# PimLb/POMDP_PBVI_Exploration

Measured on AMD Instinct MI355X. Metric: alpha-vector backups/sec, higher is better.
Workload: dtype f32

## Files before the change

### include/pbvi_hip.h

```cpp
#ifndef PBVI_HIP_H
#define PBVI_HIP_H

#include <stddef.h>
#include <stdint.h>

#ifdef __cplusplus
extern "C" {
#endif

typedef struct pbvi_engine pbvi_engine_t;

enum pbvi_status {
    PBVI_OK = 0,
    PBVI_EINVAL = -1,
    PBVI_ENOMEM = -2,
    PBVI_ERUNTIME = -3,
    PBVI_EUNSUPPORTED = -4
};

enum pbvi_dtype { PBVI_F32 = 0, PBVI_F64 = 1 };

enum pbvi_mode {
    PBVI_SPARSE = 0,
    PBVI_DENSE = 1
// ... 160 lines not shown
                             int32_t* out_steps , uint8_t* out_lost );

int pbvi_mdp_value_iteration(int device, int32_t S, int32_t A, int32_t R, const int32_t* reach_states,
                             const double* reach_prob, const double* exp_reward, const double* v0, double gamma,
                             double max_change_limit, int32_t horizon, double* out_rows, double* out_changes,
                             int32_t* out_iterations);

int64_t pbvi_belief_walk(pbvi_engine_t* e, const double* b0, int64_t n, const int32_t* actions, const int32_t* observations,
                         const uint8_t* restart, double* out_beliefs);
int pbvi_belief_walk_keys(pbvi_engine_t* e, int64_t n, uint64_t* out_keys);
int pbvi_engine_set_rto_f64(pbvi_engine_t* e, const double* rto);

int pbvi_set_formulation(pbvi_engine_t* e, int formulation);

int pbvi_set_f64_screen(pbvi_engine_t* e, int mode);

int pbvi_set_fused_projection(pbvi_engine_t* e, int enable);

int pbvi_set_score_split(pbvi_engine_t* e, int mode);

int pbvi_set_gamma_tiling(pbvi_engine_t* e, int mode, int64_t chunk_rows);
int pbvi_gamma_tiling_plan(int32_t S, int32_t A, int32_t O, int64_t V, int64_t B, int dtype, int64_t budget_bytes,
                           int64_t* chunk_rows, int64_t* n_chunks, int64_t* bytes_needed);

int pbvi_set_tie_window(pbvi_engine_t* e, double rel);

int pbvi_debug_poison(int enable);
int64_t pbvi_debug_alloc_limit(int64_t mb);
int pbvi_engine_after_oom(pbvi_engine_t* e);
int64_t pbvi_debug_live_bytes(void);

int pbvi_debug_gemm_dense(int enable);
int pbvi_debug_split_schedule(int schedule);
int64_t pbvi_debug_slabs(pbvi_engine_t* e, void* out, int64_t cap_bytes);
int pbvi_debug_slabs_fill(pbvi_engine_t* e, int byte);
int pbvi_debug_score_probe(pbvi_engine_t* e, int enable);
int pbvi_debug_score_probe_fetch(pbvi_engine_t* e, int64_t* dims, double* scalars, double* score, double* mag, double* E,
                                 int32_t* best_v, double* best_score, int32_t* queue, uint8_t* dead, int32_t* perm);
int pbvi_debug_refine_counts(pbvi_engine_t* e, int64_t out[8]);
int pbvi_debug_value_max_route(pbvi_engine_t* e, int64_t out[8]);

int64_t pbvi_device_bytes(const pbvi_engine_t* e);

#ifdef __cplusplus
}
#endif
#endif
```

### pomdp_pbvi_exploration_amd/csrc/engine.hip

```cpp
#include <algorithm>
#include <atomic>
#include <cmath>
#include <cstddef>
#include <cstdio>
#include <cstdlib>
#include <cstring>
#include <condition_variable>
#include <mutex>
#include <new>
#include <string>
#include <thread>
#include <unistd.h>
#include <vector>

#include "backup_kernels.h"
#include "split_bf16.h"
#include "upper_kernels.h"

namespace pbvi {

static thread_local std::string g_err;
static int g_poison = -1;
static bool poison_enabled() {
    if (g_poison < 0) g_poison = getenv("PBVI_POISON") != nullptr ? 1 : 0;
// ... 4528 lines not shown
}
int64_t pbvi_backup_unique_count(const pbvi_engine_t* e) { return (e && e->impl) ? e->impl->unique_count() : -1; }
int pbvi_backup_fetch_unique(pbvi_engine_t* e, void* out_rows, int32_t* out_index) {
    NEED(e);
    return e->impl->fetch_unique(out_rows, out_index);
}
int pbvi_backup_run_fetch(pbvi_engine_t* e, double gamma, int flags, pbvi_stats_t* stats, void* out_rows, int64_t cap_rows,
                          int32_t* out_slot, int32_t* out_index, int32_t* out_action, int32_t* out_best_alpha, uint8_t* out_keep,
                          int64_t* n_unique, int64_t* n_slots) {
    NEED(e);
    return e->impl->run_fetch(gamma, flags, stats, out_rows, cap_rows, out_slot, out_index, out_action, out_best_alpha, out_keep,
                              n_unique, n_slots);
}
int pbvi_backup_fetch_compact(pbvi_engine_t* e, void* out_rows, int32_t* out_index, int32_t* out_action,
                              int32_t* out_best_alpha, uint8_t* out_keep) {
    NEED(e);
    return e->impl->fetch_compact(out_rows, out_index, out_action, out_best_alpha, out_keep);
}
void* pbvi_host_alloc(size_t bytes) {
    void* p = nullptr;
    if (bytes == 0) return nullptr;
    if (hipHostMalloc(&p, bytes, hipHostMallocDefault) != hipSuccess) {
        (void)hipGetLastError();
        pbvi::set_error("pbvi_host_alloc: hipHostMalloc of " + std::to_string(bytes) + " bytes failed");
        return nullptr;
    }
    return p;
}
void pbvi_host_free(void* p) {
    if (p && hipHostFree(p) != hipSuccess) (void)hipGetLastError();
}
int pbvi_debug_gemm_dense(int enable) { return pbvi::set_gemm_force_dense(enable); }
int pbvi_debug_split_schedule(int schedule) { return pbvi::set_gemm_split_schedule(schedule); }
int64_t pbvi_debug_slabs(pbvi_engine_t* e, void* out, int64_t cap_bytes) {
    NEED(e);
    return e->impl->debug_slabs(out, cap_bytes);
}
int pbvi_debug_slabs_fill(pbvi_engine_t* e, int byte) {
    NEED(e);
    return e->impl->debug_slabs_fill(byte);
}
int pbvi_debug_score_probe(pbvi_engine_t* e, int enable) {
    NEED(e);
    return e->impl->debug_score_probe(enable);
}
int pbvi_debug_refine_counts(pbvi_engine_t* e, int64_t out[8]) {
    NEED(e);
    return e->impl->debug_refine_counts(out);
}
int pbvi_debug_value_max_route(pbvi_engine_t* e, int64_t out[8]) {
    NEED(e);
    return e->impl->debug_value_max_route(out);
}
int pbvi_debug_score_probe_fetch(pbvi_engine_t* e, int64_t* dims, double* scalars, double* score, double* mag, double* err,
                                 int32_t* best_v, double* best_score, int32_t* queue, uint8_t* dead, int32_t* perm) {
    NEED(e);
    return e->impl->debug_score_probe_fetch(dims, scalars, score, mag, err, best_v, best_score, queue, dead, perm);
}
int pbvi_backup(pbvi_engine_t* e, const void* beliefs, int64_t B, double gamma, int flags, void* out_alpha,
                int32_t* out_action, int32_t* out_best_alpha, uint8_t* out_keep, pbvi_stats_t* stats) {
    NEED(e);
    int rc = e->impl->beliefs_set(beliefs, B);
    if (rc) return rc;
    rc = e->impl->backup_run(gamma, flags, stats);
    if (rc) return rc;
    return e->impl->backup_fetch(out_alpha, out_action, out_best_alpha, out_keep);
// ... 262 lines not shown
```

### pomdp_pbvi_exploration_amd/csrc/gemm.hip

```cpp
#include "pbvi_common.h"
#include "split_bf16.h"

#include <cstdlib>
#include <map>
#include <mutex>

namespace pbvi {

typedef float f32x4 __attribute__((ext_vector_type(4)));
typedef float f32x16 __attribute__((ext_vector_type(16)));

constexpr int TILE_FLOATS = 256 * GEMM_BK;
constexpr int KL_IRR_BIT = 30;
constexpr int KL_MASK = (1 << KL_IRR_BIT) - 1;
constexpr int GEMM_LDS_BYTES = 4 * TILE_FLOATS * 4;

__device__ __forceinline__ void glds16(const float* g, float* l) {
    __builtin_amdgcn_global_load_lds((const __attribute__((address_space(1))) void*)g,
                                     (__attribute__((address_space(3))) void*)l, 16, 0, 0);
}

struct TileThread {
    int lane, wid, i, h, wr, wc;
    int srow[4], scol[4];
    int a_row[4], b_row[2];
    __device__ __forceinline__ void init() {
        const int tid = threadIdx.x;
        lane = tid & 63;
        wid = __builtin_amdgcn_readfirstlane(tid >> 6);
        i = lane & 31;
        h = lane >> 5;
        wr = wid >> 2;
        wc = wid & 3;
#pragma unroll
        for (int it = 0; it < 4; ++it) {
            const int c = it * 512 + tid;
// ... 613 lines not shown
}
__device__ __forceinline__ void split_read_b(const TileThread& t, const float* lds, int buf, int kk, bool lo, i32x4 (&b)[2]) {
    const uint32_t addr = lds_addr(lds + buf * 2 * TILE_FLOATS + TILE_FLOATS + t.wc * 64 * GEMM_BK) + split_lane_part(t, kk, lo);
    lds_read16(b[0], addr, 0);
    lds_read16(b[1], addr, 32 * GEMM_BK * 4);
}
#define PBVI_SPLIT_WAIT(N) "s_waitcnt lgkmcnt(" #N ")"
#define PBVI_SPLIT_A(a) "+v"(a[0]), "+v"(a[1]), "+v"(a[2]), "+v"(a[3])
#define PBVI_SPLIT_B(b) "+v"(b[0]), "+v"(b[1])
#define split_wait_ab(N, a, b)                                                            \
    do {                                                                                  \
        asm volatile(PBVI_SPLIT_WAIT(N) : PBVI_SPLIT_A(a), PBVI_SPLIT_B(b)::"memory");    \
        __builtin_amdgcn_sched_barrier(0);                                                \
    } while (0)
#define split_wait_a(N, a)                                              \
    do {                                                                \
        asm volatile(PBVI_SPLIT_WAIT(N) : PBVI_SPLIT_A(a)::"memory");   \
        __builtin_amdgcn_sched_barrier(0);                              \
    } while (0)
#define split_wait_b(N, b)                                              \
    do {                                                                \
        asm volatile(PBVI_SPLIT_WAIT(N) : PBVI_SPLIT_B(b)::"memory");   \
        __builtin_amdgcn_sched_barrier(0);                              \
    } while (0)
__device__ __forceinline__ void split_mfma8(const i32x4 (&a)[4], const i32x4 (&b)[2], f32x16 (&acc)[4][2]) {
#pragma unroll
    for (int mi = 0; mi < 4; ++mi)
#pragma unroll
        for (int ni = 0; ni < 2; ++ni)
            acc[mi][ni] = __builtin_amdgcn_mfma_f32_32x32x16_bf16(__builtin_bit_cast(bf16x8, a[mi]), __builtin_bit_cast(bf16x8, b[ni]),
                                                                  acc[mi][ni], 0, 0, 0);
}

template <int SCHED>
__device__ __forceinline__ void tile_run_split(const TileThread& t, float* lds, const float* Aplane, int lda, const float* Bblk,
                                               int ldb, bool gen, const int32_t* __restrict__ rsrow,
                                               const float* __restrict__ rtorow, const float* __restrict__ arow0,
                                               int64_t a_step, float gamma, const int* __restrict__ kl, int i0, int i1,
                                               f32x16 (&acc)[4][2]) {
    const int tid = threadIdx.x;
    const int kg = tid & 3, r0 = tid >> 2;
    f32x4 xb[2][2];
    i32x4 idx[2];
    f32x4 w[2];
    const uint32_t a_off = (uint32_t)(t.srow[0] * lda + t.scol[0]) * 4u;
    auto stage_a = [&](int buf, int entry) {
        const char* base = (const char*)(Aplane + (int64_t)(entry & KL_MASK) * GEMM_BK);
        float* la = lds + buf * 2 * TILE_FLOATS;
#pragma unroll
        for (int it = 0; it < 4; ++it)
            glds16((const float*)(base + (int64_t)it * 64 * lda * 4 + a_off), la + (it * 512 + t.wid * 64) * 4);
    };
    auto load_rows = [&](int entry) {
        const int k = (entry & KL_MASK) * GEMM_BK + kg * 8;
#pragma unroll
        for (int it = 0; it < 2; ++it) {
            const float* p = Bblk + (int64_t)(it * 128 + r0) * ldb + k;
            ld16(xb[it][0], p);
            ld16(xb[it][1], p + 4);
        }
    };
    auto indices = [&](int entry) {
        const int s = (entry & KL_MASK) * GEMM_BK + kg * 8;
        ld16i(idx[0], rsrow + s);
        ld16i(idx[1], rsrow + s + 4);
    };
    auto weights = [&](int entry) {
        const int s = (entry & KL_MASK) * GEMM_BK + kg * 8;
        ld16(w[0], rtorow + s);
        ld16(w[1], rtorow + s + 4);
    };
    auto alphas = [&](int entry) {
        if (entry >> KL_IRR_BIT) {
// ... 25 lines not shown
        float* lb = lds + buf * 2 * TILE_FLOATS + TILE_FLOATS;
        if (gen)
            split_store(lb, it * 128 + r0, kg, fused_value(gamma, w[0], xb[it][0]), fused_value(gamma, w[1], xb[it][1]));
        else
            split_store(lb, it * 128 + r0, kg, xb[it][0], xb[it][1]);
    };
    auto wait_and_store_b0 = [&](int buf) {
        if (gen)
            asm volatile("s_waitcnt vmcnt(6)" : "+v"(xb[0][0]), "+v"(xb[0][1]), "+v"(xb[1][0]), "+v"(xb[1][1]), "+v"(w[0]),
                         "+v"(w[1])::"memory");
        else
            asm volatile("s_waitcnt vmcnt(4)" : "+v"(xb[0][0]), "+v"(xb[0][1]), "+v"(xb[1][0]), "+v"(xb[1][1])::"memory");
        store_b(buf, 0);
    };
    {
        const int e0 = kl[i0];
        if (gen) {
            indices(e0);
            weights(e0);
            asm volatile("s_waitcnt vmcnt(0)" : "+v"(idx[0]), "+v"(idx[1])::"memory");
            alphas(e0);
            indices(i0 + 1 < i1 ? kl[i0 + 1] : 0);
        } else {
            load_rows(e0);
        }
        stage_a(0, e0);
        asm volatile("s_waitcnt vmcnt(0)" : "+v"(xb[0][0]), "+v"(xb[0][1]), "+v"(xb[1][0]), "+v"(xb[1][1]), "+v"(w[0]), "+v"(w[1]),
                     "+v"(idx[0]), "+v"(idx[1])::"memory");
        store_b(0, 0);
        store_b(0, 1);
    }
    int k_next = (i0 + 1 < i1) ? kl[i0 + 1] : 0;
    int k_after = (i0 + 2 < i1) ? kl[i0 + 2] : 0;
    __syncthreads();
    int buf = 0;
    for (int it = i0; it < i1; ++it) {
        int k_after2 = 0;
        const bool more = it + 1 < i1;
        if (more) {
            if (gen) {
                alphas(k_next);
                weights(k_next);
                indices(k_after);
            } else {
                load_rows(k_next);
            }
            stage_a(buf ^ 1, k_next);
            if (it + 3 < i1) k_after2 = kl[it + 3];
        }
        if constexpr (SCHED == SPLIT_SCHED_PIPELINED) {
            SplitSlots f;
            split_read_a(t, lds, buf, 0, false, f.a[0]);
            split_read_b(t, lds, buf, 0, false, f.b[0]);
            split_read_b(t, lds, buf, 0, true, f.b[1]);
            split_wait_ab(2, f.a[0], f.b[0]);
            split_mfma8(f.a[0], f.b[0], acc);
            __builtin_amdgcn_sched_barrier(0);
            split_read_a(t, lds, buf, 0, true, f.a[1]);
            split_wait_b(4, f.b[1]);
            split_mfma8(f.a[0], f.b[1], acc);
            __builtin_amdgcn_sched_barrier(0);
            split_read_a(t, lds, buf, 1, false, f.a[0]);
            split_read_b(t, lds, buf, 1, false, f.b[1]);
            split_wait_a(6, f.a[1]);
            split_mfma8(f.a[1], f.b[0], acc);
            __builtin_amdgcn_sched_barrier(0);
            split_read_b(t, lds, buf, 1, true, f.b[0]);
            split_wait_ab(2, f.a[0], f.b[1]);
            split_mfma8(f.a[0], f.b[1], acc);
            __builtin_amdgcn_sched_barrier(0);
            split_read_a(t, lds, buf, 1, true, f.a[1]);
            split_wait_b(4, f.b[0]);
            if (more) wait_and_store_b0(buf ^ 1);
            split_mfma8(f.a[0], f.b[0], acc);
            __builtin_amdgcn_sched_barrier(0);
            split_wait_a(0, f.a[1]);
            if (more) store_b(buf ^ 1, 1);
            split_mfma8(f.a[1], f.b[1], acc);
        } else {
            SplitFrag f;
            split_group(t, lds, buf, 0, 0, f, acc);
            split_group(t, lds, buf, 0, 1, f, acc);
            split_group(t, lds, buf, 0, 2, f, acc);
            split_group(t, lds, buf, 1, 0, f, acc);
            if (more) wait_and_store_b0(buf ^ 1);
            split_group(t, lds, buf, 1, 1, f, acc);
            if (more) store_b(buf ^ 1, 1);
            split_group(t, lds, buf, 1, 2, f, acc);
        }
        asm volatile("s_waitcnt vmcnt(0)" : "+v"(idx[0]), "+v"(idx[1])::"memory");
        __syncthreads();
        buf ^= 1;
        k_next = k_after;
        k_after = k_after2;
    }
}

template <int SCHED>
__device__ __forceinline__ void gemm_split_streamk_body(const float* __restrict__ A, int lda, const float* __restrict__ B, int ldb,
                                                        FusedB fb, SlabOut out, StreamKView v) {
    extern __shared__ __attribute__((aligned(16))) float lds[];
    streamk_walk(v, out, [&](const TileThread& t, int p, int tm, int tn, int lo, int hi, auto& acc) {
        const float* Ablk = A + (int64_t)tm * 256 * lda;
        if (fb.mat == nullptr || fb.mat[tn]) {
            const int bt = (fb.mat != nullptr && fb.ctile != nullptr) ? fb.ctile[tn] : tn;
            tile_run_split<SCHED>(t, lds, Ablk, lda, B + (int64_t)bt * 256 * ldb, ldb, false, nullptr, nullptr, nullptr, 0,
                                  0.f, v.klist + (int64_t)p * v.k_tiles, lo, hi, acc);
        } else {
            const int r0 = tn * 256;
            const int g = r0 / fb.V, v0 = r0 - g * fb.V;
            tile_run_split<SCHED>(t, lds, Ablk, lda, nullptr, 0, true, fb.rs + (int64_t)(g / fb.O) * fb.S_pad,
                                  fb.rto + (int64_t)g * fb.S_pad, fb.alpha + (int64_t)(v0 + (threadIdx.x >> 2)) * fb.lda,
                                  (int64_t)128 * fb.lda, fb.gamma, v.klist + (int64_t)p * v.k_tiles, lo, hi, acc);
        }
    });
}

__global__ __launch_bounds__(512) void k_gemm_split_streamk(
    const float* __restrict__ A, int lda, const float* __restrict__ B, int ldb, FusedB fb, float* __restrict__ C, int ldc,
    int64_t slab_stride, int tiles_m, int pairs, int k_tiles, const int* __restrict__ klist, const int* __restrict__ kcount,
    const int* __restrict__ prefix, const int* __restrict__ start_pair, const int* __restrict__ first_block,
    const int* __restrict__ plan, int ovh) {
    gemm_split_streamk_body<SPLIT_SCHED_PARENT>(A, lda, B, ldb, fb, SlabOut{C, ldc, slab_stride},
        StreamKView{klist, kcount, prefix, start_pair, first_block, plan, tiles_m, pairs, k_tiles, ovh});
}
__global__ __launch_bounds__(512) void k_gemm_split_streamk_pipelined(
    const float* __restrict__ A, int lda, const float* __restrict__ B, int ldb, FusedB fb, float* __restrict__ C, int ldc,
    int64_t slab_stride, int tiles_m, int pairs, int k_tiles, const int* __restrict__ klist, const int* __restrict__ kcount,
    const int* __restrict__ prefix, const int* __restrict__ start_pair, const int* __restrict__ first_block,
    const int* __restrict__ plan, int ovh) {
    gemm_split_streamk_body<SPLIT_SCHED_PIPELINED>(A, lda, B, ldb, fb, SlabOut{C, ldc, slab_stride},
        StreamKView{klist, kcount, prefix, start_pair, first_block, plan, tiles_m, pairs, k_tiles, ovh});
}

__global__ void k_split_probe(float* out) {
    const int lane = threadIdx.x, r = lane & 31, h = lane >> 5;
    float a[8] = {0.f, 0.f, 0.f, 0.f, 0.f, 0.f, 0.f, 0.f}, b[8] = {0.f, 0.f, 0.f, 0.f, 0.f, 0.f, 0.f, 0.f};
    const float x = 0x1.02p-120f + 0x1p-132f;
    if (h == 0) {
        a[0] = x;
        a[1] = 0x1p-100f;
        if (r == 0) b[0] = 1.f;
        if (r == 1) b[1] = 0x1p-30f;
    }
    i32x4 ah, al, bh, bl;
    uint32_t hh, ll;
#pragma unroll
    for (int p = 0; p < 4; ++p) {
        split_pair(a[2 * p], a[2 * p + 1], hh, ll); ah[p] = (int)hh; al[p] = (int)ll;
        split_pair(b[2 * p], b[2 * p + 1], hh, ll); bh[p] = (int)hh; bl[p] = (int)ll;
    }
    f32x16 acc;
#pragma unroll
    for (int e = 0; e < 16; ++e) acc[e] = 0.f;
    acc = __builtin_amdgcn_mfma_f32_32x32x16_bf16(__builtin_bit_cast(bf16x8, ah), __builtin_bit_cast(bf16x8, bh), acc, 0, 0, 0);
    acc = __builtin_amdgcn_mfma_f32_32x32x16_bf16(__builtin_bit_cast(bf16x8, ah), __builtin_bit_cast(bf16x8, bl), acc, 0, 0, 0);
    acc = __builtin_amdgcn_mfma_f32_32x32x16_bf16(__builtin_bit_cast(bf16x8, al), __builtin_bit_cast(bf16x8, bh), acc, 0, 0, 0);
    if (lane < 2) out[lane] = acc[0];
    if (lane == 0) out[2] = x;
}

int gemm_split_supported(int device) {
    static std::mutex mu;
    static std::map<int, int> known;
// ... 70 lines not shown
            if (nzB == nullptr) {
                f = 1;
            } else if (G == 0) {
                f = nzB[((int64_t)batch * tiles_n + tn) * k_tiles + kt];
            } else {
                for (int g = g0; g <= g1; ++g) f |= nzB[(int64_t)g * k_tiles + kt];
            }
        }
        const unsigned long long mask = __ballot(f);
        if (lane == 0) wcount[wid] = __popcll(mask);
        __syncthreads();
        int off = total;
        for (int w = 0; w < wid; ++w) off += wcount[w];
        if (f) {
            int entry = kt;
            if (irr != nullptr && g0 == g1 && g1 < G && irr[(int64_t)(g0 / groups_per_action) * k_tiles + kt]) entry |= 1 << KL_IRR_BIT;
            klist[(int64_t)pair * k_tiles + off + __popcll(mask & ((1ull << lane) - 1ull))] = entry;
        }
        __syncthreads();
        if (tid == 0) total += wcount[0] + wcount[1] + wcount[2] + wcount[3];
        __syncthreads();
    }
    if (tid == 0) {
        kcount[pair] = total;
        nchunks[pair] = (total + chunk_len - 1) / chunk_len;
    }
}

struct GemmEnv {
    int dense;
    int chunk;
    int no_streamk;
    int ovh;
};
static int env_int(const char* name, int dflt) { return getenv(name) ? atoi(getenv(name)) : dflt; }
static const GemmEnv& gemm_env() {
    static const GemmEnv env{env_int("PBVI_GEMM_DENSE", 0) != 0, env_int("PBVI_GEMM_CHUNK", 0), env_int("PBVI_GEMM_NO_STREAMK", 0),
                             env_int("PBVI_STREAMK_OVH", 1)};
    return env;
}

static int g_force_dense = -1;
int gemm_force_dense() { return g_force_dense < 0 ? gemm_env().dense : g_force_dense; }
int set_gemm_force_dense(int enable) {
    const int prev = gemm_force_dense();
    g_force_dense = enable ? 1 : 0;
    return prev;
}

static int g_split_schedule = SPLIT_SCHED_PARENT;
int set_gemm_split_schedule(int schedule) {
    const int prev = g_split_schedule;
    if (schedule == SPLIT_SCHED_PARENT || schedule == SPLIT_SCHED_PIPELINED) g_split_schedule = schedule;
    return prev;
}

int choose_chunk_len(int tiles_mn, int k_tiles) {
    if (const int v = gemm_env().chunk; v > 0) return v < k_tiles ? v : k_tiles;
    const int64_t total = (int64_t)tiles_mn * k_tiles;
    int64_t len = total / (256 * 8);
    if (len < 8) len = 8;
    if (len > 96) len = 96;
    if (len > k_tiles) len = k_tiles;
    return (int)len;
}

static int device_cu_count() {
    static int cus = 0;
    if (cus == 0) {
        int dev = 0;
        hipDeviceProp_t prop;
        if (hipGetDevice(&dev) == hipSuccess && hipGetDeviceProperties(&prop, dev) == hipSuccess)
            cus = prop.multiProcessorCount;
        if (cus <= 0) cus = 256;
    }
    return cus;
}

hipError_t launch_tile_nonzero_f32(const float* X, int ld, int rows_pad, int k_tiles, uint8_t* nz, hipStream_t stream) {
    dim3 grid((k_tiles + 7) / 8, rows_pad / 256);
    hipLaunchKernelGGL(k_tile_nonzero, grid, dim3(256), 0, stream, X, ld, k_tiles, nz);
    return hipGetLastError();
}

using StreamKKernel = void (*)(const float*, int, const float*, int, FusedB, float*, int, int64_t, int, int, int, const int*,
                               const int*, const int*, const int*, const int*, const int*, int);
struct StreamKKernelRow {
    int split, schedule, fused, R;
    StreamKKernel kernel;
    int lds_bytes;
};
constexpr int ANY = -1;
static const StreamKKernelRow STREAMK_KERNELS[] = {
    {1, SPLIT_SCHED_PARENT, ANY, ANY, k_gemm_split_streamk, GEMM_LDS_BYTES},
    {1, SPLIT_SCHED_PIPELINED, ANY, ANY, k_gemm_split_streamk_pipelined, GEMM_LDS_BYTES},
    {0, ANY, 0, ANY, k_gemm_nt_f32_streamk, GEMM_LDS_BYTES},
    {0, ANY, 1, 1, k_gemm_nt_f32_streamk_fused, GEMM_LDS_BYTES},
    {0, ANY, 1, 2, k_gemm_nt_f32_streamk_fused_r<2>, GEMM_LDS_BYTES_R},
    {0, ANY, 1, 3, k_gemm_nt_f32_streamk_fused_r<3>, GEMM_LDS_BYTES_R},
    {0, ANY, 1, 4, k_gemm_nt_f32_streamk_fused_r<4>, GEMM_LDS_BYTES_R},
    {0, ANY, 1, 5, k_gemm_nt_f32_streamk_fused_r<5>, GEMM_LDS_BYTES_R},
    {0, ANY, 1, 6, k_gemm_nt_f32_streamk_fused_r<6>, GEMM_LDS_BYTES_R},
    {0, ANY, 1, 7, k_gemm_nt_f32_streamk_fused_r<7>, GEMM_LDS_BYTES_R},
};
static const StreamKKernelRow* streamk_kernel(int split, int schedule, int fused, int R) {
    auto fits = [](int want, int have) { return want == ANY || want == have; };
    for (const StreamKKernelRow& row : STREAMK_KERNELS)
        if (fits(row.split, split) && fits(row.schedule, schedule) && fits(row.fused, fused) && fits(row.R, R)) return &row;
    return nullptr;
}

static hipError_t set_lds_attr() {
    static bool done = false;
    if (done) return hipSuccess;
    hipError_t e = hipFuncSetAttribute((const void*)k_gemm_nt_f32_mfma, hipFuncAttributeMaxDynamicSharedMemorySize,
                                       GEMM_LDS_BYTES);
    for (const StreamKKernelRow& row : STREAMK_KERNELS)
        if (e == hipSuccess) e = hipFuncSetAttribute((const void*)row.kernel, hipFuncAttributeMaxDynamicSharedMemorySize, row.lds_bytes);
    done = e == hipSuccess;
    return e;
}

static hipError_t build_klists(const GemmArgs& a, int batch, const FusedB* fused, hipStream_t ls) {
    if (batch < 1 || batch > 65535) return hipErrorInvalidValue;
    const GemmPlan& pl = a.plan;
    hipLaunchKernelGGL(k_build_klists, dim3(pl.tiles_m * pl.tiles_n, batch), dim3(256), 0, ls, a.nzA, a.nzB, a.G, a.v_group,
                       a.n_rows, pl.tiles_m, pl.k_tiles, pl.chunk_len, gemm_force_dense(), a.klist, a.kcount, a.nchunks,
                       fused != nullptr ? fused->irr : nullptr, fused != nullptr ? fused->O : 1);
    return hipGetLastError();
}

static hipError_t launch_mfma(const GemmArgs& a, int batch, int64_t batch_stride_b, int64_t batch_stride_c) {
    const GemmPlan& pl = a.plan;
    const int64_t groups = ((int64_t)pl.tiles_n * pl.max_chunks + 7) / 8 * 8;
    const int64_t total = groups * pl.tiles_m;
    if (total <= 0 || total > 0x7fffffff) return hipErrorInvalidValue;
    hipLaunchKernelGGL(k_gemm_nt_f32_mfma, dim3((unsigned)total, batch), dim3(512), GEMM_LDS_BYTES, a.stream, a.A, a.lda, a.B,
                       a.ldb, a.C, pl.ldc, pl.slab_stride, pl.tiles_m, pl.tiles_n, pl.k_tiles, pl.chunk_len, pl.max_chunks,
                       a.klist, a.kcount, batch_stride_b, batch_stride_c);
    return hipGetLastError();
}

hipError_t launch_score_gemm_f32(const ScoreGemmArgs& a) {
    hipError_t e = set_lds_attr();
    if (e != hipSuccess) return e;
    const GemmPlan& pl = a.plan;
    const int fused_R = a.fused != nullptr ? a.fused->R : 1;
    if (pl.streamk ? a.streamk_ws == nullptr : (a.fused != nullptr || a.split)) return hipErrorInvalidValue;
    if (a.split && fused_R != 1) return hipErrorInvalidValue;
    hipStream_t ls = (a.list_stream != nullptr && a.list_event != nullptr) ? a.list_stream : a.stream;
    if ((e = build_klists(a, 1, a.fused, ls)) != hipSuccess) return e;
    const int pairs = pl.tiles_m * pl.tiles_n, ovh = gemm_env().ovh;
    const StreamKWorkspace ws = streamk_workspace(pl, a.streamk_ws);
    if (pl.streamk) {
        hipLaunchKernelGGL(k_streamk_plan, dim3(1), dim3(256), 0, ls, a.kcount, pairs, pl.nblocks, pl.k_tiles, pl.max_chunks - 1,
                           ovh, ws.prefix, ws.start_pair, ws.first_block, a.nchunks, ws.plan);
        if ((e = hipGetLastError()) != hipSuccess) return e;
    }
    if (ls != a.stream) {
        if ((e = hipEventRecord(a.list_event, ls)) != hipSuccess) return e;
        if ((e = hipStreamWaitEvent(a.stream, a.list_event, 0)) != hipSuccess) return e;
    }
    if (!pl.streamk) return launch_mfma(a, 1, 0, 0);
    const StreamKKernelRow* row = streamk_kernel(a.split ? 1 : 0, g_split_schedule, a.fused != nullptr, fused_R);
    if (row == nullptr) return hipErrorInvalidValue;
    const FusedB fb = a.fused != nullptr ? *a.fused : FusedB{};
    hipLaunchKernelGGL(row->kernel, dim3(pl.nblocks), dim3(512), row->lds_bytes, a.stream, a.A, a.lda, a.B, a.ldb, fb, a.C, pl.ldc,
                       pl.slab_stride, pl.tiles_m, pairs, pl.k_tiles, a.klist, a.kcount, ws.prefix, ws.start_pair, ws.first_block,
                       ws.plan, ovh);
    return hipGetLastError();
}

hipError_t launch_batched_gemm_f32(const BatchedGemmArgs& a) {
    hipError_t e = set_lds_attr();
    if (e != hipSuccess) return e;
    if (a.plan.streamk) return hipErrorInvalidValue;
    if ((e = build_klists(a, a.batch, nullptr, a.stream)) != hipSuccess) return e;
    if (a.ev_before != nullptr && (e = hipEventRecord(a.ev_before, a.stream)) != hipSuccess) return e;
    if ((e = launch_mfma(a, a.batch, a.batch_stride_b, a.batch_stride_c)) != hipSuccess) return e;
    if (a.ev_after != nullptr && (e = hipEventRecord(a.ev_after, a.stream)) != hipSuccess) return e;
    return hipSuccess;
}

GemmPlan make_gemm_plan(int M_pad, int N_pad, int K_pad, bool single_chunk) {
    GemmPlan pl;
    pl.tiles_m = M_pad / GEMM_BM;
    pl.tiles_n = N_pad / GEMM_BN;
    pl.k_tiles = K_pad / GEMM_BK;
    pl.ldc = N_pad;
    pl.slab_stride = (int64_t)M_pad * N_pad;
    pl.streamk = !single_chunk && !gemm_env().no_streamk;
    pl.nblocks = device_cu_count();
    if (single_chunk) {
        pl.chunk_len = pl.k_tiles;
        pl.max_chunks = 1;
    } else if (pl.streamk) {
        const int max_split = 8;
// ... 47 lines not shown
```

### pomdp_pbvi_exploration_amd/csrc/pbvi_common.h

```cpp
#pragma once
#include <hip/hip_runtime.h>
#include <stdint.h>
#include <string>

#include "../../include/pbvi_hip.h"

namespace pbvi {

void set_error(const std::string& msg);

constexpr int GEMM_BM = 256;
constexpr int GEMM_BN = 256;
constexpr int GEMM_BK = 32;

inline int64_t round_up(int64_t x, int64_t m) { return (x + m - 1) / m * m; }

struct GemmPlan {
    int tiles_m, tiles_n, k_tiles, chunk_len, max_chunks, ldc;
    int64_t slab_stride;
    bool streamk;
    int nblocks;
    int64_t c_floats;
};
int set_gemm_force_dense(int enable);
int set_gemm_split_schedule(int schedule);
int gemm_force_dense();
struct StreamKWorkspace {
    int *prefix, *start_pair, *first_block, *plan;
};
inline StreamKWorkspace streamk_workspace(const GemmPlan& pl, int* ws, size_t* ints = nullptr) {
    const size_t pairs = (size_t)pl.tiles_m * pl.tiles_n;
    size_t off = 0;
    auto take = [&](size_t n) {
        int* p = ws != nullptr ? ws + off : nullptr;
        off += n;
        return p;
    };
    const StreamKWorkspace w{take(pairs + 1), take((size_t)pl.nblocks), take(pairs), take(2)};
    if (ints != nullptr) *ints = off;
    return w;
}
inline size_t streamk_workspace_ints(const GemmPlan& pl) {
    size_t n = 0;
    streamk_workspace(pl, nullptr, &n);
    return n;
}
struct FusedB {
    const float* alpha;
    int lda;
    const int32_t* rs;
    const float* rto;
    int S_pad, O, V;
    int R;
    float gamma;
    const int32_t* ctile;
    const uint8_t* mat;
    const int32_t* irr;
// ... 54 lines not shown
```

### pomdp_pbvi_exploration_amd/engine.py

```python
from __future__ import annotations

import ctypes as C
import os
from dataclasses import dataclass

import numpy as np

PKG_DIR = os.path.dirname(os.path.abspath(__file__))
LIB_PATH = os.path.join(PKG_DIR, 'libpbvi_hip.so')

PBVI_F32, PBVI_F64 = 0, 1
PBVI_SPARSE, PBVI_DENSE = 0, 1
PBVI_BELIEF_DOMINANCE = 1

EXPORTS = [
    'pbvi_version', 'pbvi_device_count', 'pbvi_last_error', 'pbvi_engine_create', 'pbvi_engine_destroy',
    'pbvi_alpha_set', 'pbvi_alpha_append', 'pbvi_alpha_count', 'pbvi_beliefs_set', 'pbvi_backup_run',
    'pbvi_backup_fetch', 'pbvi_backup_unique_count', 'pbvi_backup_fetch_unique', 'pbvi_backup_device_results',
    'pbvi_backup', 'pbvi_prune_dominated', 'pbvi_value_max',
    'pbvi_set_tie_window', 'pbvi_device_bytes',
    'pbvi_alpha_store_append', 'pbvi_alpha_select', 'pbvi_alpha_store_reset',
    'pbvi_belief_store_append', 'pbvi_beliefs_select', 'pbvi_belief_store_reset', 'pbvi_debug_poison',
    'pbvi_belief_update', 'pbvi_beliefs_advance', 'pbvi_beliefs_fetch', 'pbvi_beliefs_count',
    'pbvi_mdp_value_iteration', 'pbvi_set_formulation', 'pbvi_belief_walk', 'pbvi_engine_set_rto_f64', 'pbvi_backup_fetch_unique_keys', 'pbvi_assemble_rows',
    'pbvi_backup_fetch_exchange', 'pbvi_backup_store_unique',
    'pbvi_value_max_store', 'pbvi_belief_store_count', 'pbvi_alpha_store_count', 'pbvi_set_value_max_exact', 'pbvi_alpha_layout',
    'pbvi_belief_walk_keys', 'pbvi_backup_fetch_value_max',
    'pbvi_backup_fetch_compact', 'pbvi_host_alloc', 'pbvi_host_free', 'pbvi_debug_gemm_dense',
    'pbvi_backup_fetch_exchange_padded', 'pbvi_assemble_rows_store', 'pbvi_exchange_merge', 'pbvi_backup_run_fetch', 'pbvi_debug_alloc_limit', 'pbvi_debug_live_bytes', 'pbvi_engine_after_oom', 'pbvi_set_f64_screen', 'pbvi_set_fused_projection', 'pbvi_backup_fetch_row_hashes', 'pbvi_set_score_split',
    'pbvi_set_gamma_tiling', 'pbvi_gamma_tiling_plan', 'pbvi_q_values', 'pbvi_prune_dominated_masked',
    'pbvi_rollout', 'pbvi_infotaxis', 'pbvi_rollout_infotaxis', 'pbvi_debug_split_schedule', 'pbvi_debug_slabs',
    'pbvi_debug_slabs_fill', 'pbvi_env_set_frames', 'pbvi_env_set_table', 'pbvi_env_clear', 'pbvi_rollout_env',
    'pbvi_debug_score_probe', 'pbvi_debug_score_probe_fetch', 'pbvi_debug_refine_counts', 'pbvi_debug_value_max_route',
    'pbvi_upper_reset', 'pbvi_upper_append', 'pbvi_upper_count', 'pbvi_upper_bound', 'pbvi_upper_q',
    'pbvi_state_weights_set', 'pbvi_state_weights_clear', 'pbvi_space_aware', 'pbvi_rollout_space_aware',
]


class EngineUnavailable(RuntimeError):
    """The HIP library is missing or no GPU is visible."""


class PbviStats(C.Structure):
    _fields_ = [('ms_total', C.c_double), ('ms_project', C.c_double), ('ms_score', C.c_double),
                ('ms_argmax', C.c_double), ('ms_refine', C.c_double), ('ms_action', C.c_double),
                ('ms_assemble', C.c_double), ('ms_dominance', C.c_double), ('n_pairs', C.c_int64),
                ('n_dead', C.c_int64), ('n_refined', C.c_int64), ('n_refined_actions', C.c_int64),
                ('n_unique', C.c_int64),
                ('score_flops', C.c_int64), ('score_flops_executed', C.c_int64), ('score_tiles_dense', C.c_int64),
                ('score_tiles_run', C.c_int64), ('project_flops', C.c_int64), ('project_flops_executed', C.c_int64),
                ('split_k', C.c_int32), ('formulation', C.c_int32), ('n_refine_candidates', C.c_int64),
                ('ms_project_gemm', C.c_double), ('screened', C.c_int32), ('fused_projection', C.c_int32),
                ('score_split', C.c_int32), ('gamma_chunks', C.c_int32)]

    def as_dict(self) -> dict:
        return {name: getattr(self, name) for name, _ in self._fields_}


_lib = None


def load_library(path: str = LIB_PATH):
    global _lib
    if _lib is not None:
        return _lib
    path = os.environ.get('PBVI_LIB_PATH', path)
    if not os.path.exists(path):
        raise EngineUnavailable(f'{path} not found: build it with `python -m pomdp_pbvi_exploration_amd.build`')
    try:
        lib = C.CDLL(path)
    except OSError as e:
        raise EngineUnavailable(f'cannot load {path}: {e}') from e
    vp, i32p, u8p, f64p = C.c_void_p, C.POINTER(C.c_int32), C.POINTER(C.c_uint8), C.POINTER(C.c_double)
    sp = C.POINTER(PbviStats)
    protos = {
        'pbvi_version': (C.c_int, []),
        'pbvi_device_count': (C.c_int, []),
        'pbvi_last_error': (C.c_char_p, []),
        'pbvi_engine_create': (C.c_int, [C.POINTER(vp), C.c_int, C.c_int32, C.c_int32, C.c_int32, C.c_int32,
                                         i32p, vp, vp, C.c_int, C.c_int]),
        'pbvi_engine_destroy': (None, [vp]),
        'pbvi_alpha_set': (C.c_int, [vp, vp, C.c_int64]),
        'pbvi_alpha_append': (C.c_int, [vp, vp, C.c_int64]),
        'pbvi_alpha_count': (C.c_int64, [vp]),
        'pbvi_beliefs_set': (C.c_int, [vp, vp, C.c_int64]),
        'pbvi_backup_run': (C.c_int, [vp, C.c_double, C.c_int, sp]),
        'pbvi_backup_fetch': (C.c_int, [vp, vp, i32p, i32p, u8p]),
        'pbvi_backup_unique_count': (C.c_int64, [vp]),
        'pbvi_backup_fetch_unique': (C.c_int, [vp, vp, i32p]),
        'pbvi_backup_fetch_compact': (C.c_int, [vp, vp, i32p, i32p, i32p, u8p]),
        'pbvi_host_alloc': (vp, [C.c_size_t]),
        'pbvi_host_free': (None, [vp]),
        'pbvi_debug_gemm_dense': (C.c_int, [C.c_int]),
        'pbvi_debug_split_schedule': (C.c_int, [C.c_int]),
        'pbvi_debug_slabs': (C.c_int64, [vp, vp, C.c_int64]),
        'pbvi_debug_slabs_fill': (C.c_int, [vp, C.c_int]),
        'pbvi_debug_score_probe': (C.c_int, [vp, C.c_int]),
        'pbvi_debug_score_probe_fetch': (C.c_int, [vp] + [vp] * 10),
        'pbvi_debug_refine_counts': (C.c_int, [vp, vp]),
        'pbvi_debug_value_max_route': (C.c_int, [vp, vp]),
        'pbvi_backup_store_unique': (C.c_int64, [vp, i32p, C.c_int64]),
        'pbvi_backup_device_results': (C.c_int, [vp, C.POINTER(vp), C.POINTER(vp), C.POINTER(vp)]),
        'pbvi_backup': (C.c_int, [vp, vp, C.c_int64, C.c_double, C.c_int, vp, i32p, i32p, u8p, sp]),
        'pbvi_prune_dominated': (C.c_int, [vp, u8p]),
        'pbvi_prune_dominated_masked': (C.c_int, [vp, u8p, u8p]),
        'pbvi_value_max': (C.c_int, [vp, f64p, i32p]),
        'pbvi_value_max_store': (C.c_int, [vp, C.c_int64, f64p, i32p]),
        'pbvi_q_values': (C.c_int, [vp, C.c_double, f64p, i32p, i32p]),
        'pbvi_belief_store_count': (C.c_int64, [vp]),
        'pbvi_backup_fetch_value_max': (C.c_int, [vp, f64p]),
        'pbvi_belief_walk_keys': (C.c_int, [vp, C.c_int64, C.POINTER(C.c_uint64)]),
        'pbvi_set_value_max_exact': (C.c_int, [vp, C.c_int]),
        'pbvi_alpha_layout': (C.c_int, [vp, C.POINTER(C.c_int64), C.POINTER(C.c_int64)]),
        'pbvi_alpha_store_count': (C.c_int64, [vp]),
        'pbvi_alpha_store_append': (C.c_int64, [vp, vp, C.c_int64]),
        'pbvi_alpha_select': (C.c_int, [vp, i32p, C.c_int64]),
        'pbvi_alpha_store_reset': (C.c_int, [vp]),
        'pbvi_belief_store_append': (C.c_int64, [vp, vp, C.c_int64]),
        'pbvi_beliefs_select': (C.c_int, [vp, i32p, C.c_int64]),
        'pbvi_belief_store_reset': (C.c_int, [vp]),
        'pbvi_debug_poison': (C.c_int, [C.c_int]),
        'pbvi_belief_update': (C.c_int, [vp, i32p, i32p, vp]),
        'pbvi_beliefs_advance': (C.c_int, [vp, i32p, i32p, u8p, C.POINTER(C.c_int64)]),
        'pbvi_rollout': (C.c_int, [vp, i32p, C.c_int, C.c_double, i32p, u8p, C.c_uint64, C.c_uint64, C.c_int64,
                                   i32p, i32p, i32p, i32p]),
        'pbvi_infotaxis': (C.c_int, [vp, f64p, i32p, f64p, f64p]),
        'pbvi_rollout_infotaxis': (C.c_int, [vp, i32p, u8p, C.c_uint64, C.c_uint64, C.c_int64, i32p, i32p, i32p, i32p]),
# ... 55 lines not shown
def debug_alloc_limit(mb: int) -> int:
    return int(load_library().pbvi_debug_alloc_limit(int(mb)))


def debug_live_bytes() -> int:
    return int(load_library().pbvi_debug_live_bytes())


def gamma_tiling_plan(S: int, A: int, O: int, V: int, B: int, dtype: str = 'f32', budget_bytes: int = 0,
                      chunk_rows: int = 0) -> tuple:
    if dtype not in ('f32', 'f64'):
        raise ValueError("dtype must be 'f32' or 'f64'")
    for name, v in (('S', S), ('A', A), ('O', O)):
        if not -2**31 <= int(v) < 2**31:
            raise ValueError(f'{name} out of range')
    rows, n, need = C.c_int64(int(chunk_rows)), C.c_int64(0), C.c_int64(0)
    _check(load_library().pbvi_gamma_tiling_plan(int(S), int(A), int(O), int(V), int(B), 0 if dtype == 'f32' else 1,
                                                 int(budget_bytes), C.byref(rows), C.byref(n), C.byref(need)))
    return int(rows.value), int(n.value), int(need.value)


def debug_gemm_dense(enable: bool) -> bool:
    return bool(load_library().pbvi_debug_gemm_dense(1 if enable else 0))


SPLIT_SCHEDULES = {'parent': 0, 'pipelined': 1}


def debug_split_schedule(schedule: str) -> str:
    prev = int(load_library().pbvi_debug_split_schedule(SPLIT_SCHEDULES[schedule]))
    return {v: k for k, v in SPLIT_SCHEDULES.items()}[prev]


def device_count() -> int:
    return int(load_library().pbvi_device_count())


class _PinnedArray(np.ndarray):

    def __array_finalize__(self, obj):
        self._owner = getattr(obj, '_owner', None)


class PinnedBuffer:

    def __init__(self, nbytes: int):
        self._lib = load_library()
        self.nbytes = int(nbytes)
        self._p = self._lib.pbvi_host_alloc(self.nbytes)
        if not self._p:
            raise MemoryError((self._lib.pbvi_last_error() or b'').decode(errors='replace'))
        self._raw = (C.c_uint8 * self.nbytes).from_address(self._p)
        self._off = 0
        self._views = []

    def carve(self, shape, dtype) -> np.ndarray:
        dtype = np.dtype(dtype)
        n = int(np.prod(shape)) * dtype.itemsize
        off = (self._off + 255) // 256 * 256
        if off + n > self.nbytes:
            raise MemoryError('PinnedBuffer exhausted')
        self._off = off + n
        import weakref
        arr = np.frombuffer(self._raw, dtype=dtype, count=int(np.prod(shape)), offset=off).reshape(shape).view(_PinnedArray)
        arr._owner = self
        self._views.append(weakref.ref(arr))
# ... 982 lines not shown
```

Baseline: 669,700.

## Stagger split-bf16 GEMM wavefronts so half the waves run one k-step behind

Adds a staggered variant of the split-bf16 stream-K GEMM in which waves 4-7 preload the next k-tile and then run their store/stage/MFMA loop offset from waves 0-3. The aim is to overlap one group's global loads and LDS staging with the other group's MFMA work and so reduce pipeline bubbles at barriers. It is on by default (PBVI_NO_SPLIT_STAGGER turns it off), and a debug toggle is added. It adds register pressure and a more delicate barrier/LDS buffer protocol between the two wave groups, which could cause hazards or stalls.

```diff
diff --git a/include/pbvi_hip.h b/include/pbvi_hip.h
--- a/include/pbvi_hip.h
+++ b/include/pbvi_hip.h
@@ -216,6 +216,7 @@
 
 int pbvi_debug_gemm_dense(int enable);
 int pbvi_debug_split_schedule(int schedule);
+int pbvi_debug_split_stagger(int on);
 int64_t pbvi_debug_slabs(pbvi_engine_t* e, void* out, int64_t cap_bytes);
 int pbvi_debug_slabs_fill(pbvi_engine_t* e, int byte);
 int pbvi_debug_score_probe(pbvi_engine_t* e, int enable);
diff --git a/pomdp_pbvi_exploration_amd/csrc/engine.hip b/pomdp_pbvi_exploration_amd/csrc/engine.hip
--- a/pomdp_pbvi_exploration_amd/csrc/engine.hip
+++ b/pomdp_pbvi_exploration_amd/csrc/engine.hip
@@ -4584,6 +4584,7 @@
 }
 int pbvi_debug_gemm_dense(int enable) { return pbvi::set_gemm_force_dense(enable); }
 int pbvi_debug_split_schedule(int schedule) { return pbvi::set_gemm_split_schedule(schedule); }
+int pbvi_debug_split_stagger(int on) { return pbvi::set_gemm_split_stagger(on); }
 int64_t pbvi_debug_slabs(pbvi_engine_t* e, void* out, int64_t cap_bytes) {
     NEED(e);
     return e->impl->debug_slabs(out, cap_bytes);
diff --git a/pomdp_pbvi_exploration_amd/csrc/gemm.hip b/pomdp_pbvi_exploration_amd/csrc/gemm.hip
--- a/pomdp_pbvi_exploration_amd/csrc/gemm.hip
+++ b/pomdp_pbvi_exploration_amd/csrc/gemm.hip
@@ -2,6 +2,7 @@
 #include "split_bf16.h"
 
 #include <cstdlib>
+#include <type_traits>
 #include <map>
 #include <mutex>
 
@@ -681,13 +682,14 @@
                                                                   acc[mi][ni], 0, 0, 0);
 }
 
-template <int SCHED>
+template <int SCHED, bool STAG>
 __device__ __forceinline__ void tile_run_split(const TileThread& t, float* lds, const float* Aplane, int lda, const float* Bblk,
                                                int ldb, bool gen, const int32_t* __restrict__ rsrow,
                                                const float* __restrict__ rtorow, const float* __restrict__ arow0,
                                                int64_t a_step, float gamma, const int* __restrict__ kl, int i0, int i1,
                                                f32x16 (&acc)[4][2]) {
-    const int tid = threadIdx.x;
+    int tid = threadIdx.x;
+    if constexpr (STAG) asm volatile("" : "+v"(tid));
     const int kg = tid & 3, r0 = tid >> 2;
     f32x4 xb[2][2];
     i32x4 idx[2];
@@ -779,8 +781,61 @@
     }
     int k_next = (i0 + 1 < i1) ? kl[i0 + 1] : 0;
     int k_after = (i0 + 2 < i1) ? kl[i0 + 2] : 0;
+    int buf = 0;
+    if (STAG && t.wid >= 4) {
+        int k_after2 = (i0 + 3 < i1) ? kl[i0 + 3] : 0;
+        if (i0 + 1 < i1) {
+            if (gen) {
+                alphas(k_next);
+                weights(k_next);
+                indices(k_after);
+            } else {
+                load_rows(k_next);
+            }
+            asm volatile("s_waitcnt vmcnt(0)" : "+v"(xb[0][0]), "+v"(xb[0][1]), "+v"(xb[1][0]), "+v"(xb[1][1]), "+v"(w[0]),
+                         "+v"(w[1]), "+v"(idx[0]), "+v"(idx[1])::"memory");
+        }
+        __syncthreads();
+        int it = i0;
+        auto late_step = [&](auto store, auto load) {
+            const int k_after3 = (it + 4 < i1) ? kl[it + 4] : 0;
+            if constexpr (decltype(store)::value) {
+                store_b(buf ^ 1, 0);
+                store_b(buf ^ 1, 1);
+                stage_a(buf ^ 1, k_next);
+            }
+            if constexpr (decltype(load)::value) {
+                if (gen) {
+                    alphas(k_after);
+                    weights(k_after);
+                    indices(k_after2);
+                } else {
+                    load_rows(k_after);
+                }
+            }
+            __builtin_amdgcn_sched_barrier(0);
+            SplitFrag f;
+            split_group(t, lds, buf, 0, 0, f, acc);
+            split_group(t, lds, buf, 0, 1, f, acc);
+            split_group(t, lds, buf, 0, 2, f, acc);
+            split_group(t, lds, buf, 1, 0, f, acc);
+            split_group(t, lds, buf, 1, 1, f, acc);
+            split_group(t, lds, buf, 1, 2, f, acc);
+            asm volatile("s_waitcnt vmcnt(0)" : "+v"(xb[0][0]), "+v"(xb[0][1]), "+v"(xb[1][0]), "+v"(xb[1][1]), "+v"(w[0]),
+                         "+v"(w[1]), "+v"(idx[0]), "+v"(idx[1])::"memory");
+            __syncthreads();
+            buf ^= 1;
+            k_next = k_after;
+            k_after = k_after2;
+            k_after2 = k_after3;
+            ++it;
+        };
+        while (it + 2 < i1) late_step(std::true_type{}, std::true_type{});
+        if (it + 1 < i1) late_step(std::true_type{}, std::false_type{});
+        late_step(std::false_type{}, std::false_type{});
+        return;
+    }
     __syncthreads();
-    int buf = 0;
     for (int it = i0; it < i1; ++it) {
         int k_after2 = 0;
         const bool more = it + 1 < i1;
@@ -843,7 +898,7 @@
     }
 }
 
-template <int SCHED>
+template <int SCHED, bool STAG>
 __device__ __forceinline__ void gemm_split_streamk_body(const float* __restrict__ A, int lda, const float* __restrict__ B, int ldb,
                                                         FusedB fb, SlabOut out, StreamKView v) {
     extern __shared__ __attribute__((aligned(16))) float lds[];
@@ -851,12 +906,12 @@
         const float* Ablk = A + (int64_t)tm * 256 * lda;
         if (fb.mat == nullptr || fb.mat[tn]) {
             const int bt = (fb.mat != nullptr && fb.ctile != nullptr) ? fb.ctile[tn] : tn;
-            tile_run_split<SCHED>(t, lds, Ablk, lda, B + (int64_t)bt * 256 * ldb, ldb, false, nullptr, nullptr, nullptr, 0,
+            tile_run_split<SCHED, STAG>(t, lds, Ablk, lda, B + (int64_t)bt * 256 * ldb, ldb, false, nullptr, nullptr, nullptr, 0,
                                   0.f, v.klist + (int64_t)p * v.k_tiles, lo, hi, acc);
         } else {
             const int r0 = tn * 256;
             const int g = r0 / fb.V, v0 = r0 - g * fb.V;
-            tile_run_split<SCHED>(t, lds, Ablk, lda, nullptr, 0, true, fb.rs + (int64_t)(g / fb.O) * fb.S_pad,
+            tile_run_split<SCHED, STAG>(t, lds, Ablk, lda, nullptr, 0, true, fb.rs + (int64_t)(g / fb.O) * fb.S_pad,
                                   fb.rto + (int64_t)g * fb.S_pad, fb.alpha + (int64_t)(v0 + (threadIdx.x >> 2)) * fb.lda,
                                   (int64_t)128 * fb.lda, fb.gamma, v.klist + (int64_t)p * v.k_tiles, lo, hi, acc);
         }
@@ -868,7 +923,7 @@
     int64_t slab_stride, int tiles_m, int pairs, int k_tiles, const int* __restrict__ klist, const int* __restrict__ kcount,
     const int* __restrict__ prefix, const int* __restrict__ start_pair, const int* __restrict__ first_block,
     const int* __restrict__ plan, int ovh) {
-    gemm_split_streamk_body<SPLIT_SCHED_PARENT>(A, lda, B, ldb, fb, SlabOut{C, ldc, slab_stride},
+    gemm_split_streamk_body<SPLIT_SCHED_PARENT, false>(A, lda, B, ldb, fb, SlabOut{C, ldc, slab_stride},
         StreamKView{klist, kcount, prefix, start_pair, first_block, plan, tiles_m, pairs, k_tiles, ovh});
 }
 __global__ __launch_bounds__(512) void k_gemm_split_streamk_pipelined(
@@ -876,7 +931,16 @@
     int64_t slab_stride, int tiles_m, int pairs, int k_tiles, const int* __restrict__ klist, const int* __restrict__ kcount,
     const int* __restrict__ prefix, const int* __restrict__ start_pair, const int* __restrict__ first_block,
     const int* __restrict__ plan, int ovh) {
-    gemm_split_streamk_body<SPLIT_SCHED_PIPELINED>(A, lda, B, ldb, fb, SlabOut{C, ldc, slab_stride},
+    gemm_split_streamk_body<SPLIT_SCHED_PIPELINED, false>(A, lda, B, ldb, fb, SlabOut{C, ldc, slab_stride},
+        StreamKView{klist, kcount, prefix, start_pair, first_block, plan, tiles_m, pairs, k_tiles, ovh});
+}
+
+__global__ __launch_bounds__(512) void k_gemm_split_streamk_staggered(
+    const float* __restrict__ A, int lda, const float* __restrict__ B, int ldb, FusedB fb, float* __restrict__ C, int ldc,
+    int64_t slab_stride, int tiles_m, int pairs, int k_tiles, const int* __restrict__ klist, const int* __restrict__ kcount,
+    const int* __restrict__ prefix, const int* __restrict__ start_pair, const int* __restrict__ first_block,
+    const int* __restrict__ plan, int ovh) {
+    gemm_split_streamk_body<SPLIT_SCHED_PARENT, true>(A, lda, B, ldb, fb, SlabOut{C, ldc, slab_stride},
         StreamKView{klist, kcount, prefix, start_pair, first_block, plan, tiles_m, pairs, k_tiles, ovh});
 }
 
@@ -1013,11 +1077,12 @@
     int chunk;
     int no_streamk;
     int ovh;
+    int no_stagger;
 };
 static int env_int(const char* name, int dflt) { return getenv(name) ? atoi(getenv(name)) : dflt; }
 static const GemmEnv& gemm_env() {
     static const GemmEnv env{env_int("PBVI_GEMM_DENSE", 0) != 0, env_int("PBVI_GEMM_CHUNK", 0), env_int("PBVI_GEMM_NO_STREAMK", 0),
-                             env_int("PBVI_STREAMK_OVH", 1)};
+                             env_int("PBVI_STREAMK_OVH", 1), env_int("PBVI_NO_SPLIT_STAGGER", 0) != 0};
     return env;
 }
 
@@ -1033,6 +1098,14 @@
 int set_gemm_split_schedule(int schedule) {
     const int prev = g_split_schedule;
     if (schedule == SPLIT_SCHED_PARENT || schedule == SPLIT_SCHED_PIPELINED) g_split_schedule = schedule;
+    return prev;
+}
+
+static int g_split_stagger = -1;
+static int gemm_split_stagger() { return g_split_stagger < 0 ? !gemm_env().no_stagger : g_split_stagger; }
+int set_gemm_split_stagger(int on) {
+    const int prev = gemm_split_stagger();
+    g_split_stagger = on ? 1 : 0;
     return prev;
 }
 
@@ -1067,27 +1140,29 @@
 using StreamKKernel = void (*)(const float*, int, const float*, int, FusedB, float*, int, int64_t, int, int, int, const int*,
                                const int*, const int*, const int*, const int*, const int*, int);
 struct StreamKKernelRow {
-    int split, schedule, fused, R;
+    int split, schedule, stagger, fused, R;
     StreamKKernel kernel;
     int lds_bytes;
 };
 constexpr int ANY = -1;
 static const StreamKKernelRow STREAMK_KERNELS[] = {
-    {1, SPLIT_SCHED_PARENT, ANY, ANY, k_gemm_split_streamk, GEMM_LDS_BYTES},
-    {1, SPLIT_SCHED_PIPELINED, ANY, ANY, k_gemm_split_streamk_pipelined, GEMM_LDS_BYTES},
-    {0, ANY, 0, ANY, k_gemm_nt_f32_streamk, GEMM_LDS_BYTES},
-    {0, ANY, 1, 1, k_gemm_nt_f32_streamk_fused, GEMM_LDS_BYTES},
-    {0, ANY, 1, 2, k_gemm_nt_f32_streamk_fused_r<2>, GEMM_LDS_BYTES_R},
-    {0, ANY, 1, 3, k_gemm_nt_f32_streamk_fused_r<3>, GEMM_LDS_BYTES_R},
-    {0, ANY, 1, 4, k_gemm_nt_f32_streamk_fused_r<4>, GEMM_LDS_BYTES_R},
-    {0, ANY, 1, 5, k_gemm_nt_f32_streamk_fused_r<5>, GEMM_LDS_BYTES_R},
-    {0, ANY, 1, 6, k_gemm_nt_f32_streamk_fused_r<6>, GEMM_LDS_BYTES_R},
-    {0, ANY, 1, 7, k_gemm_nt_f32_streamk_fused_r<7>, GEMM_LDS_BYTES_R},
+    {1, SPLIT_SCHED_PARENT, 1, ANY, ANY, k_gemm_split_streamk_staggered, GEMM_LDS_BYTES},
+    {1, SPLIT_SCHED_PARENT, 0, ANY, ANY, k_gemm_split_streamk, GEMM_LDS_BYTES},
+    {1, SPLIT_SCHED_PIPELINED, ANY, ANY, ANY, k_gemm_split_streamk_pipelined, GEMM_LDS_BYTES},
+    {0, ANY, ANY, 0, ANY, k_gemm_nt_f32_streamk, GEMM_LDS_BYTES},
+    {0, ANY, ANY, 1, 1, k_gemm_nt_f32_streamk_fused, GEMM_LDS_BYTES},
+    {0, ANY, ANY, 1, 2, k_gemm_nt_f32_streamk_fused_r<2>, GEMM_LDS_BYTES_R},
+    {0, ANY, ANY, 1, 3, k_gemm_nt_f32_streamk_fused_r<3>, GEMM_LDS_BYTES_R},
+    {0, ANY, ANY, 1, 4, k_gemm_nt_f32_streamk_fused_r<4>, GEMM_LDS_BYTES_R},
+    {0, ANY, ANY, 1, 5, k_gemm_nt_f32_streamk_fused_r<5>, GEMM_LDS_BYTES_R},
+    {0, ANY, ANY, 1, 6, k_gemm_nt_f32_streamk_fused_r<6>, GEMM_LDS_BYTES_R},
+    {0, ANY, ANY, 1, 7, k_gemm_nt_f32_streamk_fused_r<7>, GEMM_LDS_BYTES_R},
 };
-static const StreamKKernelRow* streamk_kernel(int split, int schedule, int fused, int R) {
+static const StreamKKernelRow* streamk_kernel(int split, int schedule, int stagger, int fused, int R) {
     auto fits = [](int want, int have) { return want == ANY || want == have; };
     for (const StreamKKernelRow& row : STREAMK_KERNELS)
-        if (fits(row.split, split) && fits(row.schedule, schedule) && fits(row.fused, fused) && fits(row.R, R)) return &row;
+        if (fits(row.split, split) && fits(row.schedule, schedule) && fits(row.stagger, stagger) &&
+            fits(row.fused, fused) && fits(row.R, R)) return &row;
     return nullptr;
 }
 
@@ -1143,7 +1218,7 @@
         if ((e = hipStreamWaitEvent(a.stream, a.list_event, 0)) != hipSuccess) return e;
     }
     if (!pl.streamk) return launch_mfma(a, 1, 0, 0);
-    const StreamKKernelRow* row = streamk_kernel(a.split ? 1 : 0, g_split_schedule, a.fused != nullptr, fused_R);
+    const StreamKKernelRow* row = streamk_kernel(a.split ? 1 : 0, g_split_schedule, gemm_split_stagger(), a.fused != nullptr, fused_R);
     if (row == nullptr) return hipErrorInvalidValue;
     const FusedB fb = a.fused != nullptr ? *a.fused : FusedB{};
     hipLaunchKernelGGL(row->kernel, dim3(pl.nblocks), dim3(512), row->lds_bytes, a.stream, a.A, a.lda, a.B, a.ldb, fb, a.C, pl.ldc,
diff --git a/pomdp_pbvi_exploration_amd/csrc/pbvi_common.h b/pomdp_pbvi_exploration_amd/csrc/pbvi_common.h
--- a/pomdp_pbvi_exploration_amd/csrc/pbvi_common.h
+++ b/pomdp_pbvi_exploration_amd/csrc/pbvi_common.h
@@ -23,6 +23,7 @@
     int64_t c_floats;
 };
 int set_gemm_force_dense(int enable);
+int set_gemm_split_stagger(int on);
 int set_gemm_split_schedule(int schedule);
 int gemm_force_dense();
 struct StreamKWorkspace {
diff --git a/pomdp_pbvi_exploration_amd/engine.py b/pomdp_pbvi_exploration_amd/engine.py
--- a/pomdp_pbvi_exploration_amd/engine.py
+++ b/pomdp_pbvi_exploration_amd/engine.py
@@ -29,7 +29,7 @@
     'pbvi_backup_fetch_compact', 'pbvi_host_alloc', 'pbvi_host_free', 'pbvi_debug_gemm_dense',
     'pbvi_backup_fetch_exchange_padded', 'pbvi_assemble_rows_store', 'pbvi_exchange_merge', 'pbvi_backup_run_fetch', 'pbvi_debug_alloc_limit', 'pbvi_debug_live_bytes', 'pbvi_engine_after_oom', 'pbvi_set_f64_screen', 'pbvi_set_fused_projection', 'pbvi_backup_fetch_row_hashes', 'pbvi_set_score_split',
     'pbvi_set_gamma_tiling', 'pbvi_gamma_tiling_plan', 'pbvi_q_values', 'pbvi_prune_dominated_masked',
-    'pbvi_rollout', 'pbvi_infotaxis', 'pbvi_rollout_infotaxis', 'pbvi_debug_split_schedule', 'pbvi_debug_slabs',
+    'pbvi_rollout', 'pbvi_infotaxis', 'pbvi_rollout_infotaxis', 'pbvi_debug_split_schedule', 'pbvi_debug_split_stagger', 'pbvi_debug_slabs',
     'pbvi_debug_slabs_fill', 'pbvi_env_set_frames', 'pbvi_env_set_table', 'pbvi_env_clear', 'pbvi_rollout_env',
     'pbvi_debug_score_probe', 'pbvi_debug_score_probe_fetch', 'pbvi_debug_refine_counts', 'pbvi_debug_value_max_route',
     'pbvi_upper_reset', 'pbvi_upper_append', 'pbvi_upper_count', 'pbvi_upper_bound', 'pbvi_upper_q',
@@ -93,6 +93,7 @@
         'pbvi_host_free': (None, [vp]),
         'pbvi_debug_gemm_dense': (C.c_int, [C.c_int]),
         'pbvi_debug_split_schedule': (C.c_int, [C.c_int]),
+        'pbvi_debug_split_stagger': (C.c_int, [C.c_int]),
         'pbvi_debug_slabs': (C.c_int64, [vp, vp, C.c_int64]),
         'pbvi_debug_slabs_fill': (C.c_int, [vp, C.c_int]),
         'pbvi_debug_score_probe': (C.c_int, [vp, C.c_int]),
@@ -214,6 +215,10 @@
     return {v: k for k, v in SPLIT_SCHEDULES.items()}[prev]
 
 
+def debug_split_stagger(on: bool) -> bool:
+    return bool(load_library().pbvi_debug_split_stagger(1 if on else 0))
+
+
 def device_count() -> int:
     return int(load_library().pbvi_device_count())
 
```

After: 696,200, median of 6. 1.04x the previous value.
